# sidiso/surfh

Measured on AMD Instinct MI355X. Metric: CG-iterations/sec (forward+adjoint) on 251x251x4000 cube, higher is better.
Workload: dtype f32 (storage and accumulation; products as 2-piece fp16 splits -- 3 products per fp32 product, 1 on the far tails of the spectral response -- on the 16-bit matrix cores, in the spectral-blur GEMM and in the DFT passes)

## Files before the change

### surfh_amd/csrc/dft_h2.hip

```cpp
#include "dft_h2.h"
#include "lds_attr.h"
#include <cmath>
#include <cstring>

typedef float f32x16 __attribute__((ext_vector_type(16)));
typedef float f32x2 __attribute__((ext_vector_type(2)));
typedef unsigned u32x2 __attribute__((ext_vector_type(2)));
typedef _Float16 f16x8 __attribute__((ext_vector_type(8)));

#ifndef H2_EXP
#define H2_EXP 0
#endif

namespace {

constexpr int BK = 16, RS = 16;
constexpr int PIECE = 128 * RS;
constexpr int KT = DFT_H2_KT;
constexpr int IMG_HALFS = (int)DFT_H2_IMAGE_HALFS;
constexpr int MIX_ROWS = 256;
constexpr size_t LDS_IMG = (size_t)IMG_HALFS * 2;
constexpr size_t LDS_MIX = (size_t)2 * MIX_ROWS * 2 * sizeof(float4);
#ifndef H2_WAVES
#define H2_WAVES 8
#endif
constexpr int NWAVES = H2_WAVES, NTHREADS = 64 * NWAVES;
constexpr int E_TARGET = 10, E_LIMIT = 15;

#define MFMA3(acc_, ah_, al_, bh_, bl_)                                             \
    {                                                                               \
        f32x16 c_ = acc_;                                                           \
        c_ = __builtin_amdgcn_mfma_f32_32x32x16_f16(al_, bh_, c_, 0, 0, 0);         \
        c_ = __builtin_amdgcn_mfma_f32_32x32x16_f16(ah_, bl_, c_, 0, 0, 0);         \
        c_ = __builtin_amdgcn_mfma_f32_32x32x16_f16(ah_, bh_, c_, 0, 0, 0);         \
        acc_ = c_;                                                                  \
    }

__device__ __forceinline__ void split8h(const float (&x)[8], int e, f16x8 &fh, f16x8 &fl) {
#pragma unroll
    for (int j = 0; j < 8; ++j) {
        const float xs = __builtin_amdgcn_ldexpf(x[j], e);
        const _Float16 hh = (_Float16)xs;
        fh[j] = hh;
        fl[j] = (_Float16)(xs - (float)hh);
    }
}

__device__ __forceinline__ float pair_swap(float x) {
    return __builtin_bit_cast(float, __builtin_amdgcn_update_dpp(0, __builtin_bit_cast(int, x), 0xB1, 0xF, 0xF, false));
}

template <int KIND, bool MIX>
__global__ __launch_bounds__(NTHREADS) void dft_h2_kernel(DftH2Args g, const uint4 *__restrict__ img, int kA, int NS, long NT) {
    extern __shared__ __attribute__((aligned(16))) unsigned short lds[];
    const int tid = threadIdx.x, lane = tid & 63;
    const int wave = __builtin_amdgcn_readfirstlane(tid >> 6);
    const int l31 = lane & 31, h = lane >> 5;
    constexpr int TNW = (KIND == 0) ? 16 : 32;
    constexpr int SRC_T = (KIND == 2) ? 64 : 32, DST_T = (KIND == 1) ? 64 : 32;
    const int var = (KIND == 0) ? (l31 & 1) : 0;
    const int lcol = (KIND == 0) ? (l31 >> 1) : l31;
    const int tilesX = g.N / TNW;
    const unsigned ldb4 = (unsigned)(g.ldb * 4), ldc4 = (unsigned)(g.ldc * 4);
    const unsigned c4 = (unsigned)l31 * (KIND == 2 ? 8u : 4u), d4 = (unsigned)l31 * (KIND == 1 ? 8u : 4u);
    const int nk = g.KP / BK;
    const int kin = g.Kn / 2 + 1;
    float4 *mixbuf = reinterpret_cast<float4 *>(lds + IMG_HALFS);

    {
        uint4 *l4 = reinterpret_cast<uint4 *>(lds);
        for (int i = tid; i < IMG_HALFS / 8; i += NTHREADS) l4[i] = img[i];
    }
    const int s0 = (int)((long)NS * blockIdx.x / gridDim.x), s1 = (int)((long)NS * (blockIdx.x + 1) / gridDim.x);
    int ntw = s1 - s0;
    if (ntw > 0 && (long)NWAVES * (s1 - 1) + wave >= NT) --ntw;

    const float4 *mtab = mixbuf;
    float4 tw = make_float4(0.f, 0.f, 0.f, 0.f);
    int mix_kb = -1;
#define H2_MIXTAB(kb_)                                                                                          \
    {                                                                                                           \
        float4 *mt_ = mixbuf + ((kb_) & 1) * (MIX_ROWS * 2);                                                     \
        const int ne = (g.Kn > g.KP ? g.Kn : g.KP) * 2;                                                         \
        const float msc_ = ((kb_) == 0 || 2 * (kb_) == g.mix_Nb) ? g.mhat_self : g.mhat_pair;                   \
        for (int e_ = tid; e_ < ne; e_ += NTHREADS) {                                                           \
            const int k = e_ >> 1, tp = e_ & 1;           \
            float v[4];                                                                                         \
            _Pragma("unroll") for (int i = 0; i < 4; ++i) {                                                     \
                const int t = 2 * tp + (i >> 1), c = i & 1;                                                     \
                v[i] = (t < g.T && k < g.Kn) ? g.mhat[((long)t * 2 + c) * g.PL + (long)k * g.KBP + (kb_)] : 0.f; \
            }                                                                                                   \
            mt_[e_] = make_float4(v[0] * msc_, v[1] * msc_, v[2] * msc_, v[3] * msc_);                          \
        }                                                                                                       \
        mtab = mt_;                                                                                             \
        mix_kb = (kb_);                                                                                         \
    }
#define H2_FSETUP(t_)                                                                                           \
    if (MIX) {                                                                                                  \
        const int fn0 = ((t_) % tilesX) * TNW;                                                                   \
             \
        const int kb = g.batch > 1 ? (t_) / tilesX : fn0 / g.LP;                                                \
        const int l = g.mix_l0 + (g.batch > 1 ? fn0 : fn0 % g.LP) + lcol;                                       \
        float t4[4];                                                                                            \
        _Pragma("unroll") for (int t = 0; t < 4; ++t) t4[t] = (t < g.T) ? g.tpl[(long)t * g.LP + l] : 0.f;      \
        tw = make_float4(t4[0], t4[1], t4[2], t4[3]);                                                           \
        if (kb != mix_kb) {                                                                                     \
            H2_MIXTAB(kb);                                                                                      \
            __syncthreads();                                                                                    \
        }                                                                                                       \
    }

    __amdgpu_buffer_rsrc_t R0;
#define H2_RSRC(ptr_) __builtin_amdgcn_make_buffer_rsrc((void *)(ptr_), 0, 0xFFFFFFFF, 0x00020000)
#define H2_BLOAD(v_, s_) ((H2_EXP & 8) ? __uint_as_float((v_) + (s_)) : __builtin_bit_cast(float, __builtin_amdgcn_raw_buffer_load_b32(R0, (int)(v_), (int)(s_), 0)))
#define H2_BLOAD2(v_, s_) __builtin_bit_cast(f32x2, __builtin_amdgcn_raw_buffer_load_b64(R0, (int)(v_), (int)(s_), 0))
#define H2_LSETUP(t_)                                                                                           \
    {                                                                                                           \
        const int tx = (t_) % tilesX;                                                                           \
        const long bz_ = (t_) / tilesX;                                                                         \
        R0 = H2_RSRC(g.src + bz_ * g.sB + (long)tx * SRC_T);                                                    \
    }
#define H2_LOAD(kt_)                                                                                            \
    {                                                                                                           \
        const unsigned sk = (unsigned)((kt_) * BK) * ldb4, sp = (unsigned)(g.Kn - (kt_) * BK - 8) * ldb4;       \
        const unsigned vk = (unsigned)(8 * hv) * ldb4 + c4, vp = (unsigned)(8 * (1 - hv)) * ldb4 + c4;          \
        _Pragma("unroll") for (int j = 0; j < 8; ++j) {                                                         \
            if (KIND == 2) {                                                                                    \
                const f32x2 v2 = H2_BLOAD2(vk, sk + (unsigned)j * ldb4);                                        \
                xr[j] = v2[0];                                                                                  \
                qr[j] = v2[1];                                                                                  \
            } else {                                                                                            \
                xr[j] = H2_BLOAD(vk, sk + (unsigned)j * ldb4);                                                  \
                const unsigned q = (j == 0 && (kt_) == 0) ? c4 : vp;                                            \
                qr[j] = H2_BLOAD(q, sp - (unsigned)j * ldb4);                                                   \
            }                                                                                                   \
        }                                                                                                       \
    }
#define H2_FOLD_BODY(kt_, PV_)                                                                                   \
        _Pragma("unroll") for (int j = 0; j < 8; ++j) {                                                         \
            const int k = (kt_) * BK + 8 * hv + j;                                                              \
            const bool pv = PV_;                                                                                \
            float a = xr[j], b = qr[j];                                                                         \
            if (MIX) {             \
                const float ap = pair_swap(a), bp = pair_swap(b);                                               \
                const int kp = pv ? g.Kn - k : k;                                                               \
                                 \
                const float4 m01 = mtab[2 * k], m23 = mtab[2 * k + 1], n01 = mtab[2 * kp], n23 = mtab[2 * kp + 1]; \
                const f32x2 sv = tw.x * f32x2{m01.x, m01.y} + tw.y * f32x2{m01.z, m01.w} + tw.z * f32x2{m23.x, m23.y} + tw.w * f32x2{m23.z, m23.w}; \
                const f32x2 uv = tw.x * f32x2{n01.x, n01.y} + tw.y * f32x2{n01.z, n01.w} + tw.z * f32x2{n23.x, n23.y} + tw.w * f32x2{n23.z, n23.w}; \
                a = a * sv[0] + sgv * (ap * sv[1]);                                                             \
                b = b * uv[0] + sgv * (bp * uv[1]);                                                             \
            }                                                                                                   \
            const float ev = a + (pv ? b : 0.f), od = pv ? a - b : 0.f;                                         \
            x0[j] = ev;                                                                                         \
            x1[j] = (KIND == 0) ? pair_swap(od) : od;             \
        }
#define H2_FOLD(kt_)                                                                                            \
    {                                                                                                           \
        if (KIND == 2) {                                                                                        \
            _Pragma("unroll") for (int j = 0; j < 8; ++j) {                                                     \
                x0[j] = xr[j];                                                                                  \
                x1[j] = qr[j];                                                                                  \
            }                                                                                                   \
        } else if ((kt_) >= 1 && ((kt_) + 1) * BK <= kin && (g.Kn & 1)) {                                       \
                                                             \
            H2_FOLD_BODY(kt_, true)                                                                             \
        } else {                                                                                                \
            H2_FOLD_BODY(kt_, (k >= 1) && (k < kin) && (2 * k != g.Kn))                                         \
        }                                                                                                       \
    }
#define H2_MAXEXP(p_)                                                                                           \
    {                                                                                                           \
        float m_ = 0.f;                                                                                         \
        _Pragma("unroll") for (int j = 0; j < 8; ++j) m_ = fmaxf(m_, fmaxf(fabsf(x0[j]), fabsf(x1[j])));        \
        const unsigned mu_ = __float_as_uint(m_);                                                               \
        const auto sw_ = __builtin_amdgcn_permlane32_swap(mu_, mu_, false, false);                              \
        m_ = fmaxf(m_, fmaxf(__uint_as_float(sw_[0]), __uint_as_float(sw_[1])));                                \
        p_ = __builtin_amdgcn_frexp_expf(m_);                                                                   \
    }
#define H2_MFMA(m_, kt_, acc_, bh_, bl_)                                                                        \
    {                                                                                                           \
        const unsigned short *ra = lds + ((m_) * 2 * KT + (kt_)) * PIECE + l31 * RS + 8 * (h ^ ((l31 >> 3) & 1)); \
        _Pragma("unroll") for (int mt = 0; mt < 4; ++mt) {                                                      \
            const unsigned short *p = ra + mt * 32 * RS;                                                        \
            const f16x8 ah = *reinterpret_cast<const f16x8 *>(p);                                               \
            const f16x8 al = *reinterpret_cast<const f16x8 *>(p + KT * PIECE);                                  \
            if (!(H2_EXP & 4)) MFMA3(acc_[mt], ah, al, bh_, bl_)                                                \
            else acc_[mt][0] += (float)bh_[mt] + (float)bl_[mt] + (float)ah[0] + (float)al[0];                  \
        }                                                                                                       \
    }

    int hv = h;
    const float sgv = var ? 1.f : -1.f;
    float xr[8], qr[8];
    float x0[8], x1[8];
    f16x8 c0h, c0l, c1h, c1l;
    f32x16 acc1[4], acc2[4];

    if (MIX) {
        if (ntw > 0) {
            const int t0_ = NWAVES * s0 + wave;
            const int kb0 = g.batch > 1 ? t0_ / tilesX : ((t0_ % tilesX) * TNW) / g.LP;
            H2_MIXTAB(kb0);
        }
    }
    __syncthreads();
    if (ntw <= 0) return;

    const int *vl = g.vlist;
#define H2_RT(vt_) (vl ? NWAVES * vl[(vt_) >> 3] + ((vt_) & 7) : (vt_))
    int vt = NWAVES * s0 + wave;
    const int vtend = vt + NWAVES * ntw;
    int tile = H2_RT(vt);
    int e = 0, en = 0;

    H2_LSETUP(tile);
    H2_LOAD(0);
    H2_FSETUP(tile);
    H2_FOLD(0);
    {
        int p;
        H2_MAXEXP(p);
        e = E_TARGET - p;
    }
    split8h(x0, e, c0h, c0l);
    split8h(x1, e, c1h, c1l);
    H2_LOAD(1);
    while (true) {
        asm volatile("" : "+v"(hv));
#pragma unroll
        for (int i = 0; i < 4; ++i)
#pragma unroll
            for (int r = 0; r < 16; ++r) acc1[i][r] = acc2[i][r] = 0.f;
        const bool more = vt + NWAVES < vtend;
        const int next = more ? H2_RT(vt + NWAVES) : tile;
        const int chunk_ = g.tabLP ? (int)(((long)(tile % tilesX) * TNW % g.tabLP) >> 7) : 0;
        const int nkt = g.ktab ? g.ktab[chunk_] : nk;
        const int mtn = g.rtab ? (g.rtab[chunk_] + 31) / 32 : 4;
        for (int kt = 0; kt + 1 < nkt; ++kt) {
            H2_MFMA(0, kt, acc1, c0h, c0l);
            H2_FOLD(kt + 1);
            int p;
            H2_MAXEXP(p);
            const bool need = p + e > E_LIMIT;
            en = need ? E_TARGET - p : e;
            const int d = en - e;
            if (kt + 2 < nkt) {
                H2_LOAD(kt + 2);
            } else if (more) {
                H2_LSETUP(next);
                H2_LOAD(0);
            }
            split8h(x0, en, c0h, c0l);
            H2_MFMA(1, kt, acc2, c1h, c1l);
            split8h(x1, en, c1h, c1l);
            if (__builtin_amdgcn_ballot_w64(d != 0) != 0ull) {
#pragma unroll
                for (int mt = 0; mt < 4; ++mt)
#pragma unroll
                    for (int r = 0; r < 16; ++r) {
                        acc1[mt][r] = __builtin_amdgcn_ldexpf(acc1[mt][r], d);
                        acc2[mt][r] = __builtin_amdgcn_ldexpf(acc2[mt][r], d);
                    }
            }
            e = en;
        }
        H2_MFMA(0, nkt - 1, acc1, c0h, c0l);
        if (more) {
            H2_FSETUP(next);
            H2_FOLD(0);
            int p;
            H2_MAXEXP(p);
            en = E_TARGET - p;
            H2_LOAD(1);
            split8h(x0, en, c0h, c0l);
        }
        H2_MFMA(1, nkt - 1, acc2, c1h, c1l);
        if (more) split8h(x1, en, c1h, c1l);
        {
            const int tx = tile % tilesX;
            const long bz = tile / tilesX;
            const float f = __builtin_amdgcn_ldexpf(1.f, -e - kA);
            const float e0 = f * (var ? g.e_alt[0] : g.e[0]), e1 = f * (var ? g.e_alt[1] : g.e[1]);
            const float e2 = f * (var ? g.e_alt[2] : g.e[2]), e3 = f * (var ? g.e_alt[3] : g.e[3]);
            const __amdgpu_buffer_rsrc_t W0 = H2_RSRC(g.dst + bz * g.sC + (long)tx * DST_T);
            const unsigned lo = (unsigned)(4 * h) * ldc4 + d4, lm = (unsigned)(4 * (1 - h)) * ldc4 + d4;
            unsigned sk0 = 0u, sm0 = (unsigned)(g.Rn - 4) * ldc4;
#pragma unroll
            for (int mt = 0; mt < 4; ++mt) {
                if (mt >= mtn) break;
#pragma unroll
                for (int r = 0; r < 16; ++r) {
                    const int row = mt * 32 + (r & 3) + 8 * (r >> 2) + 4 * h;
                    const float a1 = acc1[mt][r], a2 = acc2[mt][r];
                    if (row < g.rvalid && (!(H2_EXP & 2) || g.batch < 0)) {
                        if (KIND == 1) {
                            const f32x2 v2 = {e0 * a1, e3 * a2};
                            __builtin_amdgcn_raw_buffer_store_b64(__builtin_bit_cast(u32x2, v2), W0, (int)lo, (int)sk0, 0);
                        } else {
                            __builtin_amdgcn_raw_buffer_store_b32(__float_as_uint(e0 * a1 + e1 * a2), W0, (int)lo, (int)sk0, 0);
                            if (row >= 1 && 2 * row != g.Rn)
                                __builtin_amdgcn_raw_buffer_store_b32(__float_as_uint(e2 * a1 + e3 * a2), W0, (int)lm, (int)sm0, 0);
                        }
                    }
                    const unsigned st = ((r & 3) == 3) ? 5u * ldc4 : ldc4;
                    sk0 += st; sm0 -= st;
                }
            }
        }
        if (!more) break;
        e = en;
        tile = next;
        vt += NWAVES;
    }
}


__device__ __forceinline__ float wave_max(float m) {
#define H2_DPPMAX(ctrl_) m = fmaxf(m, __builtin_bit_cast(float, __builtin_amdgcn_update_dpp(0, __builtin_bit_cast(int, m), ctrl_, 0xF, 0xF, false)))
    H2_DPPMAX(0xB1);
    H2_DPPMAX(0x4E);
    H2_DPPMAX(0x141);
    H2_DPPMAX(0x140);
#undef H2_DPPMAX
    unsigned u = __float_as_uint(m);
    auto s16 = __builtin_amdgcn_permlane16_swap(u, u, false, false);
    m = fmaxf(m, fmaxf(__uint_as_float(s16[0]), __uint_as_float(s16[1])));
    u = __float_as_uint(m);
    auto s32 = __builtin_amdgcn_permlane32_swap(u, u, false, false);
    return fmaxf(m, fmaxf(__uint_as_float(s32[0]), __uint_as_float(s32[1])));
}

__global__ __launch_bounds__(NTHREADS) void dft_h2_adjmix_kernel(DftH2Args g, DftH2AdjMix am, const uint4 *__restrict__ img, int kA, int NS) {
    static_assert(NWAVES == 8, "dft_h2_adjmix_kernel: 4 column streams x 2 row halves");
    extern __shared__ __attribute__((aligned(16))) unsigned short lds[];
    constexpr int KIND = 0;
    constexpr bool MIX = false;
    const int tid = threadIdx.x, lane = tid & 63;
    const int wave = __builtin_amdgcn_readfirstlane(tid >> 6);
    const int cs = wave;
    const int rh = ((int)blockIdx.x >> 3) & 1;
    const int vb = ((int)blockIdx.x >> 4) * 8 + ((int)blockIdx.x & 7), VP = (int)gridDim.x / 2;
    const int l31 = lane & 31, h = lane >> 5;
    constexpr int TNW = 16, SRC_T = 32;
    const int lcol = l31 >> 1;
    const int tilesX = g.N / TNW;
    const unsigned ldb4 = (unsigned)(g.ldb * 4), ldh4 = (unsigned)(am.ldh * 4);
    const unsigned c4 = (unsigned)l31 * 4u;
    const int nk = g.KP / BK;
    const int kin = g.Kn / 2 + 1;
    const int kt0 = am.kt0;
    const float4 *mtab = nullptr;
    const float4 tw = make_float4(0.f, 0.f, 0.f, 0.f);
    const float sgv = 0.f;
    (void)mtab; (void)tw; (void)sgv; (void)lcol;
    {
        uint4 *l4 = reinterpret_cast<uint4 *>(lds);
        for (int i = tid; i < IMG_HALFS / 16; i += NTHREADS) {
            const int blk = i >> 7, in = i & 127;
            l4[i] = img[blk * 256 + rh * 128 + in];
        }
    }
    const int s0 = (int)((long)NS * vb / VP), s1 = (int)((long)NS * (vb + 1) / VP);
    const int ntw = s1 - s0;
    __syncthreads();
    if (ntw <= 0) return;

    __amdgpu_buffer_rsrc_t R0;
    int hv = h;
    float xr[8], qr[8];
    float x0[8], x1[8];
    f16x8 c0h, c0l, c1h, c1l;
    f32x16 acc1[2], acc2[2];
    f32x2 M[2][2][4];
#pragma unroll
    for (int i = 0; i < 2; ++i)
#pragma unroll
        for (int k = 0; k < 2; ++k)
#pragma unroll
            for (int t = 0; t < 4; ++t) M[i][k][t] = f32x2{0.f, 0.f};

#define H2_MFMA_SW(m_, kt_, acc_, bh_, bl_)                                                                     \
    {                                                                                                           \
        const unsigned short *ra = lds + ((m_) * 2 * KT + (kt_)) * (PIECE / 2) + l31 * RS + 8 * (h ^ ((l31 >> 3) & 1)); \
        _Pragma("unroll") for (int mt = 0; mt < 2; ++mt) {                                                      \
            const unsigned short *p = ra + mt * 32 * RS;                                                        \
            const f16x8 ah = *reinterpret_cast<const f16x8 *>(p);                                               \
            const f16x8 al = *reinterpret_cast<const f16x8 *>(p + KT * (PIECE / 2));                            \
            f32x16 c_ = acc_[mt];                                                                               \
            c_ = __builtin_amdgcn_mfma_f32_32x32x16_f16(bl_, ah, c_, 0, 0, 0);                                  \
            c_ = __builtin_amdgcn_mfma_f32_32x32x16_f16(bh_, al, c_, 0, 0, 0);                                  \
            c_ = __builtin_amdgcn_mfma_f32_32x32x16_f16(bh_, ah, c_, 0, 0, 0);                                  \
            acc_[mt] = c_;                                                                                      \
        }                                                                                                       \
    }
#define H2_MAXEXP_W(p_)                                                                                         \
    {                                                                                                           \
        float m_ = 0.f;                                                                                         \
        _Pragma("unroll") for (int j = 0; j < 8; ++j) m_ = fmaxf(m_, fmaxf(fabsf(x0[j]), fabsf(x1[j])));        \
        m_ = wave_max(m_);                                                                                      \
        p_ = __builtin_amdgcn_readfirstlane(__builtin_amdgcn_frexp_expf(m_));                                   \
    }
#define H2_FLUSH(kb_)                                                                                           \
    {                                                                                                           \
        const long kbs_ = am.kbstart ? (long)am.kbstart[kb_] : (long)(kb_) * (tilesX / 8);    \
        int bf = vb;                                                                                            \
        while (bf > 0 && (long)NS * bf / VP > kbs_) --bf;                          \
        const int slot = (vb - bf) * 8 + cs;                                                                    \
        float *mp = am.mpart + ((long)(kb_) * am.nslot + slot) * (256 * 8);                                     \
        _Pragma("unroll") for (int i = 0; i < 2; ++i)                                                           \
            _Pragma("unroll") for (int k = 0; k < 2; ++k) {                                                     \
                float v[8];                                                                                     \
                _Pragma("unroll") for (int t = 0; t < 4; ++t) {                                                 \
                    _Pragma("unroll") for (int c = 0; c < 2; ++c) {                                             \
                        const unsigned u = __float_as_uint(M[i][k][t][c]);                                      \
                        const auto sw_ = __builtin_amdgcn_permlane32_swap(u, u, false, false);                  \
                        v[2 * t + c] = __uint_as_float(sw_[0]) + __uint_as_float(sw_[1]);    \
                    }                                                                                           \
                    M[i][k][t] = f32x2{0.f, 0.f};                                                               \
                }                                                                                               \
                const int r = (2 * rh + i) * 32 + l31;                                                          \
                const int row = k ? g.Rn - r : r;                                                               \
                const bool ok_ = k ? (r >= 1 && r < g.rvalid && 2 * r != g.Rn) : (r < g.rvalid);                \
                if (h == 0 && slot < am.nslot && ok_) {                                                         \
                    *reinterpret_cast<float4 *>(mp + row * 8) = make_float4(v[0], v[1], v[2], v[3]);            \
                    *reinterpret_cast<float4 *>(mp + row * 8 + 4) = make_float4(v[4], v[5], v[6], v[7]);        \
                }                                                                                               \
            }                                                                                                   \
    }

    const int *avl = am.vlist;
#define H2_ART(vt_) (avl ? 8 * avl[(vt_) >> 3] + ((vt_) & 7) : (vt_))
    int vt = 8 * s0 + cs;
    const int vtend = vt + 8 * ntw;
    int tile = H2_ART(vt);
    int e = 0, en = 0;

    H2_LSETUP(tile);
    H2_LOAD(kt0);
    H2_FOLD(kt0);
    {
        int p;
        H2_MAXEXP_W(p);
        e = E_TARGET - p;
    }
    split8h(x0, e, c0h, c0l);
    split8h(x1, e, c1h, c1l);
    H2_LOAD(kt0 + 1);
    typedef float f32x4_ __attribute__((ext_vector_type(4)));
    const unsigned hb_lds = (unsigned)(size_t)lds + (unsigned)IMG_HALFS + (unsigned)wave * 12288u;
    const unsigned hc0 = (unsigned)((lane & 7) ^ ((lane >> 4) & 3)), hc1 = hc0 ^ 4u;
    const unsigned hoa0 = (unsigned)(lane >> 3) * ldh4 + hc0 * 16u, hoa1 = (unsigned)(lane >> 3) * ldh4 + hc1 * 16u;
    const unsigned hod0 = (unsigned)(7 - (lane >> 3)) * ldh4 + hc0 * 16u, hod1 = (unsigned)(7 - (lane >> 3)) * ldh4 + hc1 * 16u;
    const unsigned hrd = hb_lds + (unsigned)l31 * 128u, hsw = (unsigned)((l31 >> 1) & 7);
#define H2_HDMA(blk_, slot_, kb_, n0_)                                                                          \
    {                                                                                                           \
        const int mt = 2 * rh + ((blk_) >> 1);                                                                  \
        const bool dsc = ((blk_) & 1) != 0;                                                                     \
        const char *hp = reinterpret_cast<const char *>(am.hsrc + (long)(kb_) * am.sH + (n0_) * 2);             \
        _Pragma("unroll") for (int i = 0; i < 4; ++i) {                                                         \
             \
            const long r0 = dsc ? (long)(g.Rn - mt * 32 - 8 * i - 7) : (long)(mt * 32 + 8 * i);                 \
            unsigned off = dsc ? ((i & 1) ? hod1 : hod0) : ((i & 1) ? hoa1 : hoa0);                             \
             \
            if (dsc && mt == 0 && i == 0 && (lane >> 3) == 0) off -= ldh4;                                      \
            const char *bp = hp + r0 * (long)ldh4;                                                              \
            const unsigned la = hb_lds + (unsigned)(slot_) * 4096u + (unsigned)i * 1024u;                       \
            if (!(H2_EXP & 16))                                                                                 \
                asm volatile("s_mov_b32 m0, %2\n\ts_nop 0\n\tglobal_load_lds_dwordx4 %0, %1" ::"v"(off), "s"(bp), "s"(la) : "memory"); \
        }                                                                                                       \
    }
#define H2_HBLOCK(i_, mir_, slot_)                                                                              \
    {                                                                                                           \
        f32x4_ hq4[4];                                                                                          \
        _Pragma("unroll") for (int q = 0; q < 4; ++q) {                                                         \
            const unsigned ad = hrd + (unsigned)(slot_) * 4096u + (((unsigned)(2 * q + h)) ^ hsw) * 16u;        \
            if (H2_EXP & 16) hq4[q] = f32x4_{1.f, 0.5f, 0.25f, 2.f};                                            \
            else asm volatile("ds_read_b128 %0, %1" : "=v"(hq4[q]) : "v"(ad) : "memory");                       \
        }                                                                                                       \
        asm volatile("s_waitcnt lgkmcnt(0)" : "+v"(hq4[0]), "+v"(hq4[1]), "+v"(hq4[2]), "+v"(hq4[3])::"memory"); \
        const float c0 = f * ((mir_) ? g.e[2] : g.e[0]), c1 = f * ((mir_) ? g.e[3] : g.e[1]);                   \
        const float d0 = f * ((mir_) ? g.e_alt[2] : g.e_alt[0]), d1 = f * ((mir_) ? g.e_alt[3] : g.e_alt[1]);   \
        _Pragma("unroll") for (int q = 0; q < 4; ++q) {                                                         \
            float ta[4], tb[4];       \
            _Pragma("unroll") for (int t = 0; t < 4; ++t) {                                                     \
                const float lo0 = __builtin_bit_cast(float, __builtin_amdgcn_readlane(__builtin_bit_cast(int, tv), (4 * q) * 4 + t));     \
                const float lo1 = __builtin_bit_cast(float, __builtin_amdgcn_readlane(__builtin_bit_cast(int, tv), (4 * q + 1) * 4 + t)); \
                const float hi0 = __builtin_bit_cast(float, __builtin_amdgcn_readlane(__builtin_bit_cast(int, tv), (4 * q + 2) * 4 + t)); \
                const float hi1 = __builtin_bit_cast(float, __builtin_amdgcn_readlane(__builtin_bit_cast(int, tv), (4 * q + 3) * 4 + t)); \
                ta[t] = h ? hi0 : lo0;                                                                          \
                tb[t] = h ? hi1 : lo1;                                                                          \
            }                                                                                                   \
            const float p0 = acc1[i_][4 * q], p1 = acc1[i_][4 * q + 1], p2 = acc1[i_][4 * q + 2], p3 = acc1[i_][4 * q + 3];   \
            const float s0v = acc2[i_][4 * q], s1v = acc2[i_][4 * q + 1], s2v = acc2[i_][4 * q + 2], s3v = acc2[i_][4 * q + 3]; \
            const float yr0 = c0 * p0 + c1 * s0v, yi0 = d0 * p1 + d1 * s1v, yr1 = c0 * p2 + c1 * s2v, yi1 = d0 * p3 + d1 * s3v; \
            const f32x4_ hh = hq4[q];                                                                           \
            const f32x2 z0 = {hh[0] * yr0 + hh[1] * yi0, hh[0] * yi0 - hh[1] * yr0};                            \
            const f32x2 z1 = {hh[2] * yr1 + hh[3] * yi1, hh[2] * yi1 - hh[3] * yr1};                            \
            _Pragma("unroll") for (int t = 0; t < 4; ++t) M[i_][mir_][t] += ta[t] * z0 + tb[t] * z1;            \
        }                                                                                                       \
    }
    const bool piped = nk - kt0 >= 5;
    while (true) {
        asm volatile("" : "+v"(hv));
#pragma unroll
        for (int i = 0; i < 2; ++i)
#pragma unroll
            for (int r = 0; r < 16; ++r) acc1[i][r] = acc2[i][r] = 0.f;
        const bool more = vt + 8 < vtend;
        const int next = more ? H2_ART(vt + 8) : tile;
        const int kb = tile / tilesX;
        const long n0 = (long)(tile % tilesX) * TNW;
        for (int kt = kt0; kt + 1 < nk; ++kt) {
            H2_MFMA_SW(0, kt, acc1, c0h, c0l);
            H2_FOLD(kt + 1);
            int p;
            H2_MAXEXP_W(p);
            en = (p + e > E_LIMIT) ? E_TARGET - p : e;
            const int d = en - e;
            if (piped) {
                if (kt == kt0 + 1) { H2_HDMA(0, 0, kb, n0); }
                else if (kt == kt0 + 2) { H2_HDMA(1, 1, kb, n0); }
                else if (kt == kt0 + 3) { H2_HDMA(2, 2, kb, n0); }
            }
            if (kt + 2 < nk) {
                H2_LOAD(kt + 2);
            } else if (more) {
                H2_LSETUP(next);
                H2_LOAD(kt0);
            }
            split8h(x0, en, c0h, c0l);
            H2_MFMA_SW(1, kt, acc2, c1h, c1l);
            split8h(x1, en, c1h, c1l);
            if (d != 0) {
#pragma unroll
                for (int mt = 0; mt < 2; ++mt)
#pragma unroll
                    for (int r = 0; r < 16; ++r) {
                        acc1[mt][r] = __builtin_amdgcn_ldexpf(acc1[mt][r], d);
                        acc2[mt][r] = __builtin_amdgcn_ldexpf(acc2[mt][r], d);
                    }
            }
            e = en;
        }
        H2_MFMA_SW(0, nk - 1, acc1, c0h, c0l);
        if (more) {
            H2_FOLD(kt0);
            int p;
            H2_MAXEXP_W(p);
            en = E_TARGET - p;
            H2_LOAD(kt0 + 1);
            split8h(x0, en, c0h, c0l);
        }
        H2_MFMA_SW(1, nk - 1, acc2, c1h, c1l);
        if (more) split8h(x1, en, c1h, c1l);
        {
            const float tv = ((lane & 3) < am.T) ? am.tpl[(long)(lane & 3) * am.LPt + n0 + (lane >> 2)] : 0.f;
            const float f = __builtin_amdgcn_ldexpf(1.f, -e - kA);
            if (!piped) {
                H2_HDMA(0, 0, kb, n0); H2_HDMA(1, 1, kb, n0); H2_HDMA(2, 2, kb, n0);
                asm volatile("s_waitcnt vmcnt(0)" ::: "memory");
            }
            H2_HBLOCK(0, 0, 0);
            H2_HDMA(3, 0, kb, n0);
            H2_HBLOCK(0, 1, 1);
            H2_HBLOCK(1, 0, 2);
            asm volatile("s_waitcnt vmcnt(0)" ::: "memory");
            H2_HBLOCK(1, 1, 0);
        }
        if (!more || next / tilesX != kb) H2_FLUSH(kb);
        if (!more) break;
        e = en;
        tile = next;
        vt += 8;
    }
#undef H2_ART
#undef H2_HDMA
#undef H2_HBLOCK
#undef H2_MFMA_SW
#undef H2_MAXEXP_W
#undef H2_FLUSH
}

__global__ __launch_bounds__(256) void dft_h2_adjmix_reduce_kernel(const float *__restrict__ mpart, float *__restrict__ madj, int nslot,
                                                                   int T, int Na, int KAP, int hb, long KBP, long PL, int NS, int G, int spk,
                                                                   float out_self, float out_pair, int Nb, const float *__restrict__ prior_src,
                                                                   float prior_mu, const int *__restrict__ kbstart) {
    const int kb = blockIdx.x;
    const float osc = (kb == 0 || 2 * kb == Nb) ? out_self : out_pair;
    const float pcb = prior_src ? 2.f - 2.f * cospif(2.f * (float)kb / (float)Nb) : 0.f;
    if (kb >= hb) {
        for (int i = blockIdx.y * 256 + threadIdx.x; i < KAP * 8; i += 256 * gridDim.y) {
            const int row = i >> 3, tc = i & 7, t = tc >> 1, c = tc & 1;
            if (t < T) madj[((long)t * 2 + c) * PL + (long)row * KBP + kb] = 0.f;
        }
        return;
    }
    int bf = 0, bl = G - 1;
    const long lo = kbstart ? kbstart[kb] : (long)kb * spk, hi = kbstart ? kbstart[kb + 1] : lo + spk;
    if (hi > lo) {
        int b = (int)(((long)lo * G) / NS);
        while (b > 0 && (long)NS * b / G > lo) --b;
        while ((long)NS * (b + 1) / G <= lo) ++b;
        bf = b;
        while (b + 1 < G && (long)NS * (b + 1) / G < hi) ++b;
        bl = b;
    }
    const int ns = hi <= lo ? 0 : ((bl - bf + 1) * 8 < nslot ? (bl - bf + 1) * 8 : nslot);
    for (int i = blockIdx.y * 256 + threadIdx.x; i < KAP * 8; i += 256 * gridDim.y) {
        const int row = i >> 3, tc = i & 7, t = tc >> 1, c = tc & 1;
        if (t >= T) continue;
        float s = 0.f;
        const long o = ((long)t * 2 + c) * PL + (long)row * KBP + kb;
        if (row < Na) {
            for (int sl = 0; sl < ns; ++sl) s += mpart[((long)kb * nslot + sl) * (256 * 8) + row * 8 + tc];
            s *= osc;
            if (prior_src) s += prior_mu * (pcb + 2.f - 2.f * cospif(2.f * (float)row / (float)Na)) * prior_src[o];
        }
        madj[o] = s;
    }
}

#undef H2_MIXTAB
#undef H2_FSETUP
#undef H2_LSETUP
#undef H2_RSRC
#undef H2_BLOAD
#undef H2_BLOAD2
#undef H2_LOAD
#undef H2_FOLD
#undef H2_FOLD_BODY
#undef H2_MAXEXP
#undef H2_MFMA
#undef H2_RT

}

int dft_h2_build_image(const float *A0, const float *A1, int MP, int KP, int lda, unsigned short *img) {
    std::memset(img, 0, DFT_H2_IMAGE_HALFS * sizeof(unsigned short));
    float amax = 0.f;
    const float *A[2] = {A0, A1};
    for (int m = 0; m < 2; ++m)
        for (int r = 0; r < MP; ++r)
            for (int k = 0; k < KP; ++k) amax = std::fmax(amax, std::fabs(A[m][(size_t)r * lda + k]));
    int pa = 0;
    if (amax > 0.f) std::frexp(amax, &pa);
    const int kA = 14 - pa;
    for (int m = 0; m < 2; ++m)
        for (int r = 0; r < MP; ++r)
            for (int k = 0; k < KP; ++k) {
                const float xs = std::ldexp(A[m][(size_t)r * lda + k], kA);
                const _Float16 hh = (_Float16)xs;
                const _Float16 ll = (_Float16)(xs - (float)hh);
                const int kt = k / BK, c = (k % BK) / 8, j = k % 8;
                const size_t pos = (size_t)kt * PIECE + (size_t)r * RS + 8 * (c ^ ((r >> 3) & 1)) + j;
                unsigned short uh, ul;
                std::memcpy(&uh, &hh, 2);
                std::memcpy(&ul, &ll, 2);
                img[((size_t)(m * 2 + 0) * KT) * PIECE + pos] = uh;
                img[((size_t)(m * 2 + 1) * KT) * PIECE + pos] = ul;
            }
    return kA;
}

int launch_dft_h2(hipStream_t stream, const DftH2Args &g, const unsigned short *img, int kA) {
    if (g.kind < 0 || g.kind > 2 || g.KP % BK || g.KP < 2 * BK || g.KP > KT * BK || g.N % 128 || g.batch < 1 || !img || !g.src || !g.dst)
        return (int)hipErrorInvalidValue;
    if (g.kind != 2 && g.KP > g.Kn) return (int)hipErrorInvalidValue;
    if (g.rvalid < 1 || g.rvalid > 128) return (int)hipErrorInvalidValue;
    const double rows_src = (double)(g.Kn > g.KP ? g.Kn : g.KP) + 9.0, rows_dst = (double)(g.Rn > 128 ? g.Rn : 128) + 9.0;
    if (rows_src * (double)g.ldb * 4.0 + 1024.0 >= 4294967296.0 || rows_dst * (double)g.ldc * 4.0 + 1024.0 >= 4294967296.0) return (int)hipErrorInvalidValue;
    const int mix_rows = g.Kn > g.KP ? g.Kn : g.KP;
    if (g.mhat && (g.kind != 0 || g.LP % 128 || g.T < 1 || g.T > 4 || mix_rows > MIX_ROWS || !g.tpl)) return (int)hipErrorInvalidValue;
    static int cus_of[64] = {0};
    int dev = 0;
    if (hipGetDevice(&dev) != hipSuccess || dev < 0 || dev >= 64) return (int)hipErrorInvalidDevice;
    if (!cus_of[dev]) {
        int cus = 0;
        if (hipDeviceGetAttribute(&cus, hipDeviceAttributeMultiprocessorCount, dev) != hipSuccess) return (int)hipErrorInvalidDevice;
        cus_of[dev] = cus;
    }
    const int tnw = g.kind == 0 ? 16 : 32;
    long NT = (long)(g.N / tnw) * g.batch;
    long NS = (NT + NWAVES - 1) / NWAVES;
    if (NS >= 2147483647L / NWAVES) return (int)hipErrorInvalidValue;
    if ((g.ktab || g.rtab) && (g.tabLP < 128 || g.tabLP % 128)) return (int)hipErrorInvalidValue;
    if (g.vlist) {
        if (NT % NWAVES || g.nvalid < 1 || g.nvalid > NS) return (int)hipErrorInvalidValue;
        NS = g.nvalid;
        NT = NS * NWAVES;
    }
    dim3 grid((unsigned)(NS < cus_of[dev] ? NS : cus_of[dev]));
    const uint4 *im = reinterpret_cast<const uint4 *>(img);
    static unsigned long long d0 = 0, d1 = 0, d2 = 0, d3 = 0;
    if (g.mhat) {
        if (int e = ensure_dynamic_lds(dft_h2_kernel<0, true>, LDS_IMG + LDS_MIX, d3)) return e;
        hipLaunchKernelGGL((dft_h2_kernel<0, true>), grid, dim3(NTHREADS), LDS_IMG + LDS_MIX, stream, g, im, kA, (int)NS, NT);
    } else if (g.kind == 0) {
        if (int e = ensure_dynamic_lds(dft_h2_kernel<0, false>, LDS_IMG, d0)) return e;
        hipLaunchKernelGGL((dft_h2_kernel<0, false>), grid, dim3(NTHREADS), LDS_IMG, stream, g, im, kA, (int)NS, NT);
    } else if (g.kind == 1) {
        if (int e = ensure_dynamic_lds(dft_h2_kernel<1, false>, LDS_IMG, d1)) return e;
        hipLaunchKernelGGL((dft_h2_kernel<1, false>), grid, dim3(NTHREADS), LDS_IMG, stream, g, im, kA, (int)NS, NT);
    } else {
        if (int e = ensure_dynamic_lds(dft_h2_kernel<2, false>, LDS_IMG, d2)) return e;
        hipLaunchKernelGGL((dft_h2_kernel<2, false>), grid, dim3(NTHREADS), LDS_IMG, stream, g, im, kA, (int)NS, NT);
    }
    return (int)hipGetLastError();
}

static void adjmix_geometry(int dev_cus, long tilesX, int hb, long nvalid, long &NS, int &G, int &nslot) {
    NS = nvalid > 0 ? nvalid : tilesX / 8 * hb;
    long pairs = dev_cus / 16 * 8;
    if (pairs < 8) pairs = 8;
    while (pairs > 8 && pairs > NS) pairs -= 8;
    G = (int)(2 * pairs);
    const long spk = tilesX / 8;
    const long per = NS / pairs > 0 ? NS / pairs : 1;
    nslot = (int)(8 * ((spk + per - 1) / per + 2));
}

size_t dft_h2_adjmix_part_floats(long LP, int hb, long nvalid) {
    int dev = 0, cus = 0;
    if (hipGetDevice(&dev) != hipSuccess || hipDeviceGetAttribute(&cus, hipDeviceAttributeMultiprocessorCount, dev) != hipSuccess || cus < 1) return 0;
    long NS; int G, nslot;
    adjmix_geometry(cus, LP / 16, hb, nvalid, NS, G, nslot);
    return (size_t)hb * nslot * 256 * 8;
}

int launch_dft_h2_adjmix(hipStream_t stream, const DftH2Args &g, const DftH2AdjMix &am0, float *madj, long PL, long KBP, const unsigned short *img, int kA) {
    if (am0.kt0 < 0 || (am0.kt0 > 0 && g.KP / BK - am0.kt0 < 2)) return (int)hipErrorInvalidValue;
    if (g.kind != 0 || g.mhat || g.KP % BK || g.KP < 2 * BK || g.KP > KT * BK || g.KP > g.Kn || g.N % 128 || g.batch < 1 || !img || !g.src ||
        !am0.hsrc || !am0.tpl || !am0.mpart || !madj || am0.T < 1 || am0.T > 4 || g.Rn < 32 * 3 + 31 || g.Rn > 255 || g.rvalid < 1 || g.rvalid > 128)
        return (int)hipErrorInvalidValue;
    const double rows_src = (double)g.Kn + 9.0;
    if (rows_src * (double)g.ldb * 4.0 + 1024.0 >= 4294967296.0 || 260.0 * (double)am0.ldh * 4.0 + 1024.0 >= 4294967296.0) return (int)hipErrorInvalidValue;
    int dev = 0, cus = 0;
    if (hipGetDevice(&dev) != hipSuccess || hipDeviceGetAttribute(&cus, hipDeviceAttributeMultiprocessorCount, dev) != hipSuccess || cus < 1) return (int)hipErrorInvalidDevice;
    long NS; int G, nslot;
    if ((am0.vlist != nullptr) != (am0.kbstart != nullptr) || (am0.vlist && (am0.nvalid < 1 || am0.nvalid > (long)(g.N / 128) * g.batch)))
        return (int)hipErrorInvalidValue;
    adjmix_geometry(cus, g.N / 16, g.batch, am0.vlist ? am0.nvalid : 0, NS, G, nslot);
    if (NS >= 2147483647L / 8 || g.N % 128) return (int)hipErrorInvalidValue;
    DftH2AdjMix am = am0;
    am.nslot = nslot;
    static unsigned long long d4 = 0;
    const size_t ldsb = LDS_IMG / 2 + (size_t)NWAVES * 12288;
    if (int e = ensure_dynamic_lds(dft_h2_adjmix_kernel, ldsb, d4)) return e;
    hipLaunchKernelGGL(dft_h2_adjmix_kernel, dim3((unsigned)G), dim3(NTHREADS), ldsb, stream, g, am, reinterpret_cast<const uint4 *>(img), kA, (int)NS);
    if (hipError_t e = hipGetLastError(); e != hipSuccess) return (int)e;
    hipLaunchKernelGGL(dft_h2_adjmix_reduce_kernel, dim3((unsigned)KBP, 8), dim3(256), 0, stream, am.mpart, madj, nslot, am.T, g.Rn, (int)(PL / KBP),
                       g.batch, KBP, PL, (int)NS, G / 2, (int)(g.N / 16 / 8), am.out_self, am.out_pair, am.Nb, am.prior_src, am.prior_mu, am.kbstart);
    return (int)hipGetLastError();
}

bool dft_h2_supported(int Na, int Nb, long NAP, long KBP, long LP) {
    const double pitch = 2.0 * (double)(NAP > KBP ? NAP : KBP) * (double)LP * 4.0;
    const int n = Na > Nb ? Na : Nb, m = Na < Nb ? Na : Nb;
    return n / 2 + 1 <= 128 && m / 2 + 1 > BK && n <= MIX_ROWS && LP % 128 == 0 && ((double)n + 9.0) * pitch + 1024.0 < 4294967296.0;
}
```

Before: 359.5.

## Streamline adjmix kernel: faster fp16 split, max-exponent reduce, fold, and template broadcast

Rewrites several inner-loop helpers of the adjoint-mix DFT kernel. The fp16 hi/lo split now uses a precomputed power-of-two scale and v_fma_mixlo/mixhi to form the residual. The wave max-exponent now uses v_max3 with DPP integer max and readlanes. Folding of the even/odd halves is vectorised on interior tiles. The template broadcast now uses ds_bpermute instead of 16 readlanes and selects, with the scale factor f folded into tv. The epilogue also swaps the acc2 lane pairing. Debug H2_EXP bits add experimental fake paths, but they are off by default. The aim is fewer VALU/SALU instructions per k-step, at the cost of inline-asm rigidity and a possible change in the accumulator lane mapping.

```diff
diff --git a/surfh_amd/csrc/dft_h2.hip b/surfh_amd/csrc/dft_h2.hip
--- a/surfh_amd/csrc/dft_h2.hip
+++ b/surfh_amd/csrc/dft_h2.hip
@@ -7,6 +7,9 @@
 typedef float f32x2 __attribute__((ext_vector_type(2)));
 typedef unsigned u32x2 __attribute__((ext_vector_type(2)));
 typedef _Float16 f16x8 __attribute__((ext_vector_type(8)));
+typedef float f32x4_t __attribute__((ext_vector_type(4)));
+typedef _Float16 f16x2 __attribute__((ext_vector_type(2)));
+typedef unsigned u32x4 __attribute__((ext_vector_type(4)));
 
 #ifndef H2_EXP
 #define H2_EXP 0
@@ -329,6 +332,45 @@
     u = __float_as_uint(m);
     auto s32 = __builtin_amdgcn_permlane32_swap(u, u, false, false);
     return fmaxf(m, fmaxf(__uint_as_float(s32[0]), __uint_as_float(s32[1])));
+}
+
+__device__ __forceinline__ void split8s(const float (&x)[8], float s, f16x8 &fh, f16x8 &fl) {
+    if (H2_EXP & 256) {
+        fh = __builtin_bit_cast(f16x8, f32x4_t{x[0], x[1], x[2], x[3]});
+        fl = __builtin_bit_cast(f16x8, f32x4_t{x[4], x[5], x[6], x[7]});
+        return;
+    }
+    u32x4 hv, lv;
+#pragma unroll
+    for (int j = 0; j < 4; ++j) {
+        const f32x2 xs = f32x2{x[2 * j], x[2 * j + 1]} * s;
+        const unsigned hh = __builtin_bit_cast(unsigned, f16x2{(_Float16)xs[0], (_Float16)xs[1]});
+        unsigned lo;
+        asm("v_fma_mixlo_f16 %0, %1, %2, -%3 op_sel_hi:[0,0,1]" : "=v"(lo) : "v"(x[2 * j]), "s"(s), "v"(hh));
+        asm("v_fma_mixhi_f16 %0, %1, %2, -%3 op_sel:[0,0,1] op_sel_hi:[0,0,1]" : "+v"(lo) : "v"(x[2 * j + 1]), "s"(s), "v"(hh));
+        hv[j] = hh;
+        lv[j] = lo;
+    }
+    fh = __builtin_bit_cast(f16x8, hv);
+    fl = __builtin_bit_cast(f16x8, lv);
+}
+
+__device__ __forceinline__ int wave_exp(const float (&x0)[8], const float (&x1)[8]) {
+    float m;
+    asm("v_max3_f32 %0, |%1|, |%2|, |%3|" : "=v"(m) : "v"(x0[0]), "v"(x0[1]), "v"(x0[2]));
+#define H2_MAX3(a_, b_) asm("v_max3_f32 %0, %1, |%2|, |%3|" : "=v"(m) : "v"(m), "v"(a_), "v"(b_))
+    H2_MAX3(x0[3], x0[4]); H2_MAX3(x0[5], x0[6]); H2_MAX3(x0[7], x1[0]); H2_MAX3(x1[1], x1[2]);
+    H2_MAX3(x1[3], x1[4]); H2_MAX3(x1[5], x1[6]); H2_MAX3(x1[7], x1[7]);
+#undef H2_MAX3
+    unsigned u = __float_as_uint(m);
+    u = max(u, (unsigned)__builtin_amdgcn_mov_dpp((int)u, 0xB1, 0xF, 0xF, true));
+    u = max(u, (unsigned)__builtin_amdgcn_mov_dpp((int)u, 0x4E, 0xF, 0xF, true));
+    u = max(u, (unsigned)__builtin_amdgcn_mov_dpp((int)u, 0x141, 0xF, 0xF, true));
+    u = max(u, (unsigned)__builtin_amdgcn_mov_dpp((int)u, 0x140, 0xF, 0xF, true));
+    const unsigned r = max(max((unsigned)__builtin_amdgcn_readlane((int)u, 0), (unsigned)__builtin_amdgcn_readlane((int)u, 16)),
+                           max((unsigned)__builtin_amdgcn_readlane((int)u, 32), (unsigned)__builtin_amdgcn_readlane((int)u, 48)));
+    const int p = r ? (int)(r >> 23) - 126 : 0;
+    return p > -96 ? p : -96;
 }
 
 __global__ __launch_bounds__(NTHREADS) void dft_h2_adjmix_kernel(DftH2Args g, DftH2AdjMix am, const uint4 *__restrict__ img, int kA, int NS) {
@@ -388,18 +430,20 @@
             const f16x8 ah = *reinterpret_cast<const f16x8 *>(p);                                               \
             const f16x8 al = *reinterpret_cast<const f16x8 *>(p + KT * (PIECE / 2));                            \
             f32x16 c_ = acc_[mt];                                                                               \
-            c_ = __builtin_amdgcn_mfma_f32_32x32x16_f16(bl_, ah, c_, 0, 0, 0);                                  \
-            c_ = __builtin_amdgcn_mfma_f32_32x32x16_f16(bh_, al, c_, 0, 0, 0);                                  \
-            c_ = __builtin_amdgcn_mfma_f32_32x32x16_f16(bh_, ah, c_, 0, 0, 0);                                  \
+            if (H2_EXP & 32) {                                                                                  \
+                c_[0] += (float)bh_[mt] + (float)bl_[mt] + (float)ah[0] + (float)al[0];                         \
+            } else {                                                                                            \
+                c_ = __builtin_amdgcn_mfma_f32_32x32x16_f16(bl_, ah, c_, 0, 0, 0);                              \
+                c_ = __builtin_amdgcn_mfma_f32_32x32x16_f16(bh_, al, c_, 0, 0, 0);                              \
+                c_ = __builtin_amdgcn_mfma_f32_32x32x16_f16(bh_, ah, c_, 0, 0, 0);                              \
+            }                                                                                                   \
             acc_[mt] = c_;                                                                                      \
         }                                                                                                       \
     }
 #define H2_MAXEXP_W(p_)                                                                                         \
     {                                                                                                           \
-        float m_ = 0.f;                                                                                         \
-        _Pragma("unroll") for (int j = 0; j < 8; ++j) m_ = fmaxf(m_, fmaxf(fabsf(x0[j]), fabsf(x1[j])));        \
-        m_ = wave_max(m_);                                                                                      \
-        p_ = __builtin_amdgcn_readfirstlane(__builtin_amdgcn_frexp_expf(m_));                                   \
+        if (H2_EXP & 128) p_ = __builtin_amdgcn_readfirstlane(__float_as_int(x0[0]) >> 23) & 3;              \
+        else p_ = wave_exp(x0, x1);                                                                             \
     }
 #define H2_FLUSH(kb_)                                                                                           \
     {                                                                                                           \
@@ -429,6 +473,23 @@
             }                                                                                                   \
     }
 
+#define H2_FOLD_X(kt_)                                                                                          \
+    if (H2_EXP & 64) {                                              \
+        _Pragma("unroll") for (int j = 0; j < 8; ++j) { x0[j] = xr[j]; x1[j] = qr[j]; }                         \
+    } else if ((kt_) >= 1 && ((kt_) + 1) * BK <= kin && (g.Kn & 1)) {                                           \
+        _Pragma("unroll") for (int j = 0; j < 8; j += 2) {                                                      \
+            const f32x2 a = {xr[j], xr[j + 1]}, b = {qr[j], qr[j + 1]}, ev = a + b, od = a - b;                 \
+            x0[j] = ev[0]; x0[j + 1] = ev[1]; x1[j] = od[0]; x1[j + 1] = od[1];                                 \
+        }                                                                                                       \
+    } else {                                                                                                    \
+        _Pragma("unroll") for (int j = 0; j < 8; ++j) {                                                         \
+            const int k = (kt_) * BK + 8 * hv + j;                                                              \
+            const bool pv = (k >= 1) && (k < kin) && (2 * k != g.Kn);                                           \
+            x0[j] = xr[j] + (pv ? qr[j] : 0.f);                                                                 \
+            x1[j] = pv ? xr[j] - qr[j] : 0.f;                                                                   \
+        }                                                                                                       \
+    }
+#define H2_SCALE(e_) __uint_as_float((unsigned)((e_) + 127) << 23)
     const int *avl = am.vlist;
 #define H2_ART(vt_) (avl ? 8 * avl[(vt_) >> 3] + ((vt_) & 7) : (vt_))
     int vt = 8 * s0 + cs;
@@ -438,14 +499,14 @@
 
     H2_LSETUP(tile);
     H2_LOAD(kt0);
-    H2_FOLD(kt0);
+    H2_FOLD_X(kt0);
     {
         int p;
         H2_MAXEXP_W(p);
         e = E_TARGET - p;
     }
-    split8h(x0, e, c0h, c0l);
-    split8h(x1, e, c1h, c1l);
+    split8s(x0, H2_SCALE(e), c0h, c0l);
+    split8s(x1, H2_SCALE(e), c1h, c1l);
     H2_LOAD(kt0 + 1);
     typedef float f32x4_ __attribute__((ext_vector_type(4)));
     const unsigned hb_lds = (unsigned)(size_t)lds + (unsigned)IMG_HALFS + (unsigned)wave * 12288u;
@@ -479,25 +540,25 @@
             else asm volatile("ds_read_b128 %0, %1" : "=v"(hq4[q]) : "v"(ad) : "memory");                       \
         }                                                                                                       \
         asm volatile("s_waitcnt lgkmcnt(0)" : "+v"(hq4[0]), "+v"(hq4[1]), "+v"(hq4[2]), "+v"(hq4[3])::"memory"); \
-        const float c0 = f * ((mir_) ? g.e[2] : g.e[0]), c1 = f * ((mir_) ? g.e[3] : g.e[1]);                   \
-        const float d0 = f * ((mir_) ? g.e_alt[2] : g.e_alt[0]), d1 = f * ((mir_) ? g.e_alt[3] : g.e_alt[1]);   \
+        int tvb = tvf;              \
+        asm volatile("" : "+v"(tvb));                                                                           \
+        const float c0 = (mir_) ? g.e[2] : g.e[0], c1 = (mir_) ? g.e[3] : g.e[1];                               \
+        const float d0 = (mir_) ? g.e_alt[2] : g.e_alt[0], d1 = (mir_) ? g.e_alt[3] : g.e_alt[1];               \
         _Pragma("unroll") for (int q = 0; q < 4; ++q) {                                                         \
-            float ta[4], tb[4];       \
-            _Pragma("unroll") for (int t = 0; t < 4; ++t) {                                                     \
-                const float lo0 = __builtin_bit_cast(float, __builtin_amdgcn_readlane(__builtin_bit_cast(int, tv), (4 * q) * 4 + t));     \
-                const float lo1 = __builtin_bit_cast(float, __builtin_amdgcn_readlane(__builtin_bit_cast(int, tv), (4 * q + 1) * 4 + t)); \
-                const float hi0 = __builtin_bit_cast(float, __builtin_amdgcn_readlane(__builtin_bit_cast(int, tv), (4 * q + 2) * 4 + t)); \
-                const float hi1 = __builtin_bit_cast(float, __builtin_amdgcn_readlane(__builtin_bit_cast(int, tv), (4 * q + 3) * 4 + t)); \
-                ta[t] = h ? hi0 : lo0;                                                                          \
-                tb[t] = h ? hi1 : lo1;                                                                          \
-            }                                                                                                   \
             const float p0 = acc1[i_][4 * q], p1 = acc1[i_][4 * q + 1], p2 = acc1[i_][4 * q + 2], p3 = acc1[i_][4 * q + 3];   \
-            const float s0v = acc2[i_][4 * q], s1v = acc2[i_][4 * q + 1], s2v = acc2[i_][4 * q + 2], s3v = acc2[i_][4 * q + 3]; \
+                                                \
+            const float s0v = acc2[i_][4 * q + 1], s1v = acc2[i_][4 * q], s2v = acc2[i_][4 * q + 3], s3v = acc2[i_][4 * q + 2]; \
             const float yr0 = c0 * p0 + c1 * s0v, yi0 = d0 * p1 + d1 * s1v, yr1 = c0 * p2 + c1 * s2v, yi1 = d0 * p3 + d1 * s3v; \
             const f32x4_ hh = hq4[q];                                                                           \
+            float ta[4], tb[4];         \
+            _Pragma("unroll") for (int t = 0; t < 4; ++t) {                                                     \
+                ta[t] = (H2_EXP & 1024) ? 0.25f * t : __int_as_float(__builtin_amdgcn_ds_bpermute(tva + 4 * (16 * q + t), tvb));       \
+                tb[t] = (H2_EXP & 1024) ? 0.5f * t : __int_as_float(__builtin_amdgcn_ds_bpermute(tva + 4 * (16 * q + 4 + t), tvb));    \
+            }                                                                                                   \
             const f32x2 z0 = {hh[0] * yr0 + hh[1] * yi0, hh[0] * yi0 - hh[1] * yr0};                            \
             const f32x2 z1 = {hh[2] * yr1 + hh[3] * yi1, hh[2] * yi1 - hh[3] * yr1};                            \
-            _Pragma("unroll") for (int t = 0; t < 4; ++t) M[i_][mir_][t] += ta[t] * z0 + tb[t] * z1;            \
+            if (H2_EXP & 512) M[i_][mir_][q] += f32x2{hh[0] + p0 + s0v, hh[1] + p1 + s1v};                   \
+            else _Pragma("unroll") for (int t = 0; t < 4; ++t) M[i_][mir_][t] += ta[t] * z0 + tb[t] * z1; \
         }                                                                                                       \
     }
     const bool piped = nk - kt0 >= 5;
@@ -511,9 +572,10 @@
         const int next = more ? H2_ART(vt + 8) : tile;
         const int kb = tile / tilesX;
         const long n0 = (long)(tile % tilesX) * TNW;
+        const float tv = ((lane & 3) < am.T) ? am.tpl[(long)(lane & 3) * am.LPt + n0 + (lane >> 2)] : 0.f;
         for (int kt = kt0; kt + 1 < nk; ++kt) {
             H2_MFMA_SW(0, kt, acc1, c0h, c0l);
-            H2_FOLD(kt + 1);
+            H2_FOLD_X(kt + 1);
             int p;
             H2_MAXEXP_W(p);
             en = (p + e > E_LIMIT) ? E_TARGET - p : e;
@@ -529,9 +591,10 @@
                 H2_LSETUP(next);
                 H2_LOAD(kt0);
             }
-            split8h(x0, en, c0h, c0l);
+            const float sc = H2_SCALE(en);
+            split8s(x0, sc, c0h, c0l);
             H2_MFMA_SW(1, kt, acc2, c1h, c1l);
-            split8h(x1, en, c1h, c1l);
+            split8s(x1, sc, c1h, c1l);
             if (d != 0) {
 #pragma unroll
                 for (int mt = 0; mt < 2; ++mt)
@@ -545,18 +608,19 @@
         }
         H2_MFMA_SW(0, nk - 1, acc1, c0h, c0l);
         if (more) {
-            H2_FOLD(kt0);
+            H2_FOLD_X(kt0);
             int p;
             H2_MAXEXP_W(p);
             en = E_TARGET - p;
             H2_LOAD(kt0 + 1);
-            split8h(x0, en, c0h, c0l);
+            split8s(x0, H2_SCALE(en), c0h, c0l);
         }
         H2_MFMA_SW(1, nk - 1, acc2, c1h, c1l);
-        if (more) split8h(x1, en, c1h, c1l);
+        if (more) split8s(x1, H2_SCALE(en), c1h, c1l);
         {
-            const float tv = ((lane & 3) < am.T) ? am.tpl[(long)(lane & 3) * am.LPt + n0 + (lane >> 2)] : 0.f;
             const float f = __builtin_amdgcn_ldexpf(1.f, -e - kA);
+            const int tvf = __float_as_int(tv * f);
+            const int tva = 32 * h;
             if (!piped) {
                 H2_HDMA(0, 0, kb, n0); H2_HDMA(1, 1, kb, n0); H2_HDMA(2, 2, kb, n0);
                 asm volatile("s_waitcnt vmcnt(0)" ::: "memory");
@@ -580,6 +644,7 @@
 #undef H2_MFMA_SW
 #undef H2_MAXEXP_W
 #undef H2_FLUSH
+#undef H2_FOLD_X
 }
 
 __global__ __launch_bounds__(256) void dft_h2_adjmix_reduce_kernel(const float *__restrict__ mpart, float *__restrict__ madj, int nslot,
```

Measured after the change: 360.9, median of 6. About the same (+0.4%).
